# askerlee/AdaFace-dev

Measured on AMD Instinct MI355X. Metric: denoise-steps/sec SD-1.5 U-Net 512px bs=4/GPU, higher is better.
Workload: dtype f16; 1 GPU; adaface_txt2img_ddim: SD-1.5 U-Net eps-prediction + CFG + DDIM update, 512x512 (latent 64x64), bs=4/GPU, U-Net batch 8 (cond+uncond), 77 tokens, DDIM-50 timesteps, random-init weights; parallelism=replicas x1, hipgraph=True, finite=True

## Files before the change

### adaface-dev_amd/csrc/af_gemm.hip

```cpp
#include "af_common.h"

int af_gemm_n_major(int M, int N, int K, int cin) { return (long)N * K > (long)M * cin ? 1 : 0; }

namespace {

struct GemmDev {
  const half_t* a1;
  const half_t* a2;
  const half_t* wt;
  const float* bias;
  const half_t* rowbias;
  const half_t* residual;
  half_t* out;
  half_t* out2;
  int M, N, K, kpad;
  int c1, c2, lda1, lda2;
  int H, W, Ho, Wo, HoWo, Heff, Weff, stride, upsample;
  int rows_per_batch, ld_rowbias, act_silu, ld_out, split_col, ld_out2;
  int tiles_n, tiles_m, n_major;
  int tap_shift;
  int splits, kt_per_split;
  float* ws;
  int* counters;
  int out_f32;
  int wpf, wpf_coop;
};

constexpr int BK = 64;
enum { EPI_STD = 0, EPI_GEGLU = 1, EPI_SPLIT_T = 2 };

template <int BM, int BN, int TAPS, int EPI, bool FAST = false>
__global__ __launch_bounds__(256, 2) void af_gemm_kernel(GemmDev p) {
  constexpr int WM = BM / 2, WN = BN / 2;
  constexpr int TM = WM / 16, TN = WN / 16;
  constexpr int AI = BM / 32, WI = BN / 32;
  constexpr int STAGE = (BM + BN) * BK;
  extern __shared__ __attribute__((aligned(16))) char af_smem[];
  half_t* lds = reinterpret_cast<half_t*>(af_smem);

  const int tid = threadIdx.x, lane = tid & 63, wave = tid >> 6;
  const int wm = wave & 1, wn = wave >> 1;

  int tile_m, tile_n;
  {
    const int nwg = gridDim.x, bid = blockIdx.x;
    const int q = nwg >> 3, r = nwg & 7, xcd = bid & 7, idx = bid >> 3;
    const int lid = (xcd < r ? xcd * (q + 1) : r * (q + 1) + (xcd - r) * q) + idx;
    if (p.n_major) {
// ... 408 lines not shown
         ((uintptr_t)d->bias & 15) == 0 && (((uintptr_t)d->rowbias | (uintptr_t)d->residual) & 7) == 0 && d->ld_rowbias % 4 == 0 &&
         ((uintptr_t)d->out & (d->out_mode == AF_OUT_F32 ? 15 : 7)) == 0;
}

static int launch_direct(const GemmDev& p0, hipStream_t stream) {
  GemmDev p = p0;
  p.tiles_m = (p.M + 31) / 32;
  p.tiles_n = (p.N + 63) / 64;
  p.splits = 1;
  const dim3 grid(p.tiles_m * p.tiles_n), block(256);
  if ((p.kpad >> 5) % 4 == 0) hipLaunchKernelGGL(af_gemm_direct_kernel<4>, grid, block, 0, stream, p);
  else hipLaunchKernelGGL(af_gemm_direct_kernel<2>, grid, block, 0, stream, p);
  return af_check_launch("af_gemm(tile 18)");
}

__global__ __launch_bounds__(256) void af_splitk_reduce_kernel(GemmDev p) {
  const long i4 = (long)blockIdx.x * 256 + threadIdx.x;
  const int n4 = p.N >> 2;
  if (i4 >= (long)p.M * n4) return;
  const int m = (int)(i4 / n4);
  const int n0 = (int)(i4 - (long)m * n4) * 4;
  floatx4 v = {0.f, 0.f, 0.f, 0.f};
  for (int sp = 0; sp < p.splits; ++sp) v += *reinterpret_cast<const floatx4*>(p.ws + ((size_t)sp * p.M + m) * p.N + n0);
  if (p.bias) v += *reinterpret_cast<const floatx4*>(p.bias + n0);
  if (p.rowbias) {
    const half4_t rv = *reinterpret_cast<const half4_t*>(p.rowbias + (size_t)(m / p.rows_per_batch) * p.ld_rowbias + n0);
#pragma unroll
    for (int i = 0; i < 4; ++i) v[i] += (float)rv[i];
  }
  if (p.act_silu == 1) {
#pragma unroll
    for (int i = 0; i < 4; ++i) v[i] = af_silu(v[i]);
  } else if (p.act_silu == 3) {
#pragma unroll
    for (int i = 0; i < 4; ++i) v[i] = v[i] * af_sigmoid(1.702f * v[i]);
  }
  if (p.residual) {
    const half4_t rv = *reinterpret_cast<const half4_t*>(p.residual + (size_t)m * p.N + n0);
#pragma unroll
    for (int i = 0; i < 4; ++i) v[i] += (float)rv[i];
  }
  if (p.out_f32) {
    *reinterpret_cast<floatx4*>(reinterpret_cast<float*>(p.out) + (size_t)m * p.ld_out + n0) = v;
    return;
  }
  const half4_t h = {(half_t)v[0], (half_t)v[1], (half_t)v[2], (half_t)v[3]};
// ... 48 lines not shown
  if (cpg <= 0 || cpg % 2 != 0 || bn % cpg != 0 || N % cpg != 0 || N / cpg > 32 || N % bn != 0 || N % 8 != 0) return 0;
  if (rows_per_batch <= 0 || rows_per_batch % 128 != 0 || rows_per_batch / 128 > 128) return 0;
  return 1;
}

extern "C" int af_gemm(const af_gemm_desc* d, void* stream) {
  AF_REQUIRE(d != nullptr, "af_gemm: null descriptor");
  AF_REQUIRE(d->a1 && d->wt && d->out, "af_gemm: a1/wt/out must be non-null");
  AF_REQUIRE(d->M > 0 && d->N > 0 && d->K > 0, "af_gemm: M, N, K must be positive");
  AF_REQUIRE(d->taps == 1 || d->taps == 9, "af_gemm: taps must be 1 or 9");
  AF_REQUIRE(d->kpad % BK == 0 && d->kpad >= d->K, "af_gemm: kpad must be a multiple of 64 and >= K");
  AF_REQUIRE(d->N % 4 == 0, "af_gemm: N must be a multiple of 4");
  AF_REQUIRE(d->c1 > 0 && d->c1 % 8 == 0 && d->c2 >= 0 && d->c2 % 8 == 0, "af_gemm: c1/c2 must be multiples of 8");
  AF_REQUIRE(d->c2 == 0 || d->a2 != nullptr, "af_gemm: a2 is null but c2 > 0");
  const bool ktail = d->c3 > 0 || d->c4 > 0;
  if (ktail) {
    AF_REQUIRE(d->taps == 9 && d->c3 > 0 && d->a3 != nullptr && d->c4 >= 0 && (d->c4 == 0 || d->a4 != nullptr), "af_gemm: the K tail needs taps == 9 and a3 (a4 when c4 > 0)");
    AF_REQUIRE(d->c3 % 64 == 0 && d->c4 % 64 == 0, "af_gemm: c3 / c4 must be multiples of 64");
    AF_REQUIRE((d->lda3 == 0 || (d->lda3 >= d->c3 && d->lda3 % 8 == 0)) && (d->lda4 == 0 || (d->lda4 >= d->c4 && d->lda4 % 8 == 0)), "af_gemm: bad lda3 / lda4");
    AF_REQUIRE((d->stride == 0 || d->stride == 1) && d->upsample == 0 && d->tap_shift == 0, "af_gemm: the K tail needs stride 1, no upsample, no tap_shift");
    AF_SUPPORTED((d->tile >= 7 && d->tile <= 15), "af_gemm: the K tail runs on the whole-line tiles 7 .. 13, 15 and the halo-resident tile 14 only");
  }
  if (d->upsample == 3) {
    AF_SUPPORTED(d->tile == 14 && af_gemm_halo_variant(d) == 4, "af_gemm: upsample = 3 (phase form) runs on tile 14 inside af_gemm_halo_variant's scope only");
    AF_REQUIRE(d->zeros != nullptr, "af_gemm: zeros must be non-null");
    AfLaunchScope scope(AF_FAM_GEMM, stream);
    AF_SUPPORTED(af_gemm3_try_launch(d, 1, 11, (hipStream_t)stream) == 0, "af_gemm: upsample = 3 needs a 16-byte aligned output with ld_out % 8 == 0");
    return af_check_launch("af_gemm(tile 14, phase form)");
  }
  AF_REQUIRE(d->K == d->taps * (d->c1 + d->c2) + d->c3 + d->c4, "af_gemm: K != taps*(c1+c2) (+ c3 + c4)");
  const bool gnp = d->gn_partials != nullptr;
  if (gnp) {
    const int rpb = d->rows_per_batch > 0 ? d->rows_per_batch : d->M;
    AF_SUPPORTED(af_gemm_gn_stats_ok(d->tile, d->splits, d->taps, d->act, d->out_mode, d->N, d->gn_cpg, rpb) == 1,
                 "af_gemm: gn_partials needs a whole-line tile whose width is a multiple of gn_cpg, the standard fp16 epilogue, whole 128-row tiles per "
                 "batch item and no split-K (af_gemm_gn_stats_ok)");
    AF_REQUIRE(d->M % rpb == 0 && (d->ld_out == 0 || d->ld_out == d->N) && ((uintptr_t)d->out & 15) == 0, "af_gemm: gn_partials needs M = B * rows_per_batch and a dense, 16-byte aligned output");
  }
  GemmDev p;
  p.a1 = (const half_t*)d->a1;
  p.a2 = (const half_t*)d->a2;
  p.wt = (const half_t*)d->wt;
  p.bias = (const float*)d->bias;
  p.rowbias = (const half_t*)d->rowbias;
  p.residual = (const half_t*)d->residual;
  p.out = (half_t*)d->out;
  p.out2 = (half_t*)d->out2;
  p.M = d->M;
// ... 2 lines not shown
  p.kpad = d->kpad;
  p.c1 = d->c1;
  p.c2 = d->c2;
  p.lda1 = d->lda1 ? d->lda1 : d->c1;
  p.lda2 = d->lda2 ? d->lda2 : d->c2;
  p.stride = d->stride ? d->stride : 1;
  p.upsample = d->upsample;
  p.H = d->H;
  p.W = d->W;
  p.Ho = d->Ho;
  p.Wo = d->Wo;
  p.HoWo = d->Ho * d->Wo;
  p.Heff = p.upsample ? 2 * d->H : d->H;
  p.Weff = p.upsample ? 2 * d->W : d->W;
  if (p.upsample == 2 && d->taps == 9) {
    p.Heff = d->Ho;
    p.Weff = d->Wo;
  }
  p.rows_per_batch = d->rows_per_batch > 0 ? d->rows_per_batch : d->M;
  p.ld_rowbias = d->ld_rowbias;
  p.act_silu = d->act == AF_ACT_SILU ? 1 : (d->act == AF_ACT_QUICKGELU ? 3 : 0);
  p.split_col = d->split_col;
  p.ld_out2 = d->ld_out2;
  p.tiles_n = 0;
  p.tap_shift = d->taps == 9 ? d->tap_shift : 0;
  p.splits = d->splits > 1 ? d->splits : 1;
  p.kt_per_split = 0;
  p.ws = (float*)d->workspace;
  p.counters = (d->splitk_fused && d->workspace && d->workspace_bytes > AF_SPLITK_COUNTER_BYTES)
                   ? reinterpret_cast<int*>(static_cast<char*>(d->workspace) + d->workspace_bytes - AF_SPLITK_COUNTER_BYTES) : nullptr;
  if (d->taps == 9) {
    AF_REQUIRE(d->B > 0 && d->H > 0 && d->W > 0 && d->Ho > 0 && d->Wo > 0, "af_gemm: conv geometry missing");
    AF_REQUIRE(p.stride == 1 || p.stride == 2, "af_gemm: stride must be 1 or 2");
    AF_REQUIRE(p.upsample >= 0 && p.upsample <= 2, "af_gemm: upsample must be 0, 1 (nearest) or 2 (zero-insert)");
    AF_REQUIRE(!(p.upsample && p.stride != 1), "af_gemm: upsample requires stride 1");
    AF_REQUIRE(d->M == d->B * d->Ho * d->Wo, "af_gemm: M != B*Ho*Wo");
    if (p.upsample == 2)
      AF_REQUIRE((d->Ho == 2 * d->H || d->Ho == 2 * d->H - 1) && (d->Wo == 2 * d->W || d->Wo == 2 * d->W - 1),
                 "af_gemm: zero-insert mode needs Ho in {2H, 2H-1}, Wo in {2W, 2W-1}");
    AF_REQUIRE(d->Ho == (p.Heff + 2 - 3) / p.stride + 1 && d->Wo == (p.Weff + 2 - 3) / p.stride + 1,
               "af_gemm: Ho/Wo inconsistent with H/W/stride/upsample");
  }
  if (d->rowbias) AF_REQUIRE(d->ld_rowbias >= d->N, "af_gemm: ld_rowbias < N");
  const bool geglu = d->act == AF_ACT_GEGLU;
  if (geglu) {
    AF_REQUIRE(d->N % 32 == 0, "af_gemm: GEGLU needs N % 32 == 0 (interleaved 16-row groups)");
// ... 61 lines not shown
```

### adaface-dev_amd/csrc/af_gemm3.hip

```cpp
#include <algorithm>

#include "af_common.h"

int af_gemm_n_major(int M, int N, int K, int cin);

namespace {

struct Gemm3Dev {
  const half_t* a1;
  const half_t* a2;
  const half_t* wt;
  const half_t* zeros;
  const float* bias;
  const half_t* rowbias;
  const half_t* residual;
  half_t* out;
  half_t* out2;
  int split_col, ld_out2;
  int M, N, K, kpad, npad;
  int c1, c2, lda1, lda2;
  const half_t* a3;
  const half_t* a4;
  int c3, c4, lda3, lda4;
  int H, W, Ho, Wo, HoWo, stride;
// ... 724 lines not shown
    const int row = (wave * WPW + j) * 8 + prow;
    const int n = min(tile_n * BN + row, p.npad - 1);
    w_off[j] = ((unsigned)n * (unsigned)p.kpad + (unsigned)((slot ^ ((row >> 1) & 7)) * 8)) * 2u;
  }
  unsigned a_off1[APW], a_off2[APW];
  const half_t* a_px1[APW];
  const half_t* a_px2[APW];
#pragma unroll
  for (int j = 0; j < APW; ++j) {
    const int row = (wave * APW + j) * 8 + prow;
    const int mc = min(tile_m * BM + row, p.M - 1);
    const unsigned ch = (unsigned)(a_lc[j] * 8);
    if constexpr (TAPS == 9) {
      a_off1[j] = ((unsigned)mc * (unsigned)p.lda3 + ch) * 2u;
      a_off2[j] = ((unsigned)mc * (unsigned)p.lda4 + ch) * 2u;
      a_px1[j] = p.a1 + (size_t)a_base[j] * p.c1 + ch;
      a_px2[j] = p.a2 + (size_t)a_base[j] * p.c2 + ch;
    } else {
      a_off1[j] = ((unsigned)mc * (unsigned)p.lda1 + ch) * 2u;
      a_off2[j] = ((unsigned)mc * (unsigned)p.lda2 + ch) * 2u;
    }
  }

  auto issue_stage = [&](int kt, int sl) {
    char* As = af_smem + sl * STAGE;
    char* Ws = As + BM * 128;
    const int k0 = kt * BKW;
    if constexpr (TAPS == 9) {
      if (p.upsample) {
        const int tp = k0 / Cin;
        const int c0 = k0 - tp * Cin;
        const bool first = c0 < p.c1;
        const half_t* src = first ? p.a1 : p.a2;
        const int cs = first ? p.c1 : p.c2;
        const int coff = first ? c0 : c0 - p.c1;
        const int ty = tp / 3, tx = tp - ty * 3;
#pragma unroll
        for (int j = 0; j < APW; ++j) {
          const bool ok = (a_mask[j] >> tp) & 1u;
          const int dpix = (((a_par[j] & 1) + ty - 1) >> 1) * p.W + (((a_par[j] >> 1) + tx - 1) >> 1);
          const half_t* g = ok ? src + (size_t)(a_base[j] + dpix) * cs + coff + a_lc[j] * 8 : p.zeros;
          glds16(g, As + (wave * APW + j) * 1024);
        }
#pragma unroll
        for (int j = 0; j < WPW; ++j) glds16(wok[j] ? wptr[j] + k0 : p.zeros, Ws + (wave * WPW + j) * 1024);
        return;
      }
    }
    if (TAPS == 9 && p.c3 > 0 && k0 >= 9 * Cin) {
      const int kt0 = k0 - 9 * Cin;
      const bool first = kt0 < p.c3;
      const half_t* sb = first ? p.a3 + kt0 : p.a4 + (kt0 - p.c3);
      if (first) {
#pragma unroll
        for (int j = 0; j < APW; ++j) glds16_sbase(sb, a_off1[j], As + (wave * APW + j) * 1024);
      } else {
#pragma unroll
        for (int j = 0; j < APW; ++j) glds16_sbase(sb, a_off2[j], As + (wave * APW + j) * 1024);
      }
    } else if constexpr (TAPS == 9) {
      const int tp = k0 / Cin;
      const int c0 = k0 - tp * Cin;
      const bool first = c0 < p.c1;
      const int cs = first ? p.c1 : p.c2;
      const int ty = tp / 3, tx = tp - ty * 3;
      const long soff = (long)((ty - 1) * p.W + (tx - 1)) * cs + (first ? c0 : c0 - p.c1);
#pragma unroll
      for (int j = 0; j < APW; ++j) {
        const bool ok = (a_mask[j] >> tp) & 1u;
        const half_t* px = a_px1[j];
        if (!first) px = a_px2[j];
        const half_t* g = ok ? px + soff : p.zeros;
        glds16(g, As + (wave * APW + j) * 1024);
      }
    } else {
      const bool first = k0 < p.c1;
      const half_t* sb = first ? p.a1 + k0 : p.a2 + (k0 - p.c1);
      if (first) {
#pragma unroll
        for (int j = 0; j < APW; ++j) glds16_sbase(sb, a_off1[j], As + (wave * APW + j) * 1024);
      } else {
#pragma unroll
        for (int j = 0; j < APW; ++j) glds16_sbase(sb, a_off2[j], As + (wave * APW + j) * 1024);
      }
    }
// ... 741 lines not shown
      mfmas();
      __builtin_amdgcn_s_setprio(1);
      tb = tn_;
    }
    asm volatile("s_waitcnt vmcnt(0)" ::: "memory");
    __builtin_amdgcn_s_barrier();
  }
  __builtin_amdgcn_s_setprio(0);
  gemm3_epilogue<E3_STD, NWM, NWN, TN, CH_LDS, UP2 ? 2 : (PATCH ? 1 : 0)>(p, acc, af_smem, tile_m, tile_n, wm, wn, fr, fq, tid);
}

static bool conv3h_up2_ok(const af_gemm_desc* d) {
  if (d->taps != 9 || d->tap_shift || (d->stride ? d->stride : 1) != 1 || d->c1 <= 0 || d->c1 % 64 != 0 || d->c2 || d->c3 || d->c4) return false;
  if (d->N <= 0 || d->N % CH_BN != 0 || d->K != 4 * d->c1 || d->kpad % 64 != 0 || d->kpad < d->K) return false;
  if ((d->W != 16 && d->W != 32) || d->H <= 0 || d->B <= 0 || (d->H * d->W) % CH_BM != 0 || d->Ho != 2 * d->H || d->Wo != 2 * d->W) return false;
  if ((long)d->M != (long)d->B * d->Ho * d->Wo || d->splits > 1) return false;
  if (d->act == AF_ACT_GEGLU || d->out_mode != AF_OUT_NORMAL || d->ln_colsum != nullptr) return false;
  if (d->rowbias != nullptr || d->residual != nullptr || d->gn_partials != nullptr) return false;
  if ((long)d->B * d->H * d->W * d->c1 * 2 >= (1L << 32)) return false;
  if ((long)((4L * d->N + 127) / 128 * 128) * d->kpad * 2 >= (1L << 32)) return false;
  return true;
}

static int conv3h_variant(const af_gemm_desc* d) {
  if (d->upsample == 3) return conv3h_up2_ok(d) ? 4 : 0;
  if (d->taps != 9 || (d->upsample != 0 && d->upsample != 1) || d->tap_shift || d->c1 % 64 != 0 || d->c2 % 64 != 0) return 0;
  const bool n160 = d->N % CH_BN == 0;
  if (!n160 && d->N % 128 != 0) return 0;
  if (d->c3 || d->c4) {
    if (!n160 || d->c3 <= 0 || d->c3 % 64 != 0 || d->c4 < 0 || d->c4 % 64 != 0 || d->upsample) return 0;
    if ((long)d->M * std::max(d->lda3 ? d->lda3 : d->c3, d->lda4 ? d->lda4 : d->c4) * 2 >= (1L << 32)) return 0;
    if ((long)d->B * d->H * d->W >= (1L << 24)) return 0;
  }
  const int up = d->upsample ? 2 : 1;
  if ((d->stride ? d->stride : 1) != 1 || d->Ho != up * d->H || d->Wo != up * d->W) return 0;
  if (d->M % CH_BM != 0 || d->M != d->B * d->Ho * d->Wo) return 0;
  if (d->act == AF_ACT_GEGLU || d->out_mode == AF_OUT_SPLIT_T || d->ln_colsum != nullptr || d->kpad % 64 != 0) return 0;
  if ((long)d->B * d->H * d->W * std::max(d->c1, d->c2) * 2 >= (1L << 32)) return 0;
  if ((long)((d->N + 127) / 128 * 128) * d->kpad * 2 >= (1L << 32)) return 0;
  if (d->Wo > 64) {
    if (n160 || d->Wo % 16 != 0 || d->Ho % 16 != 0 || d->c3 || d->c4 || d->splits > 1) return 0;
    return 3;
  }
  if (d->Wo != 8 && d->Wo != 16 && d->Wo != 32 && d->Wo != 64) return 0;
  const int rows = CH_BM / d->Wo;
  if (d->Ho % rows != 0 && rows % d->Ho != 0) return 0;
  if (d->Ho < rows && (rows / d->Ho) * (d->Ho + 2) * (d->Wo + 2) > CH_NP_MAX * 8) return 0;
  return n160 ? 1 : 2;
// ... 288 lines not shown
          for (int tm = 0; tm < TM; ++tm) xf[tm] = *reinterpret_cast<const half8_t*>(As + (wm * 64 + tm * 16) * 128 + rd);
#pragma unroll
          for (int tn = 0; tn < 5; ++tn)
#pragma unroll
            for (int tm = 0; tm < TM; ++tm) acc3[tn][tm] = __builtin_amdgcn_mfma_f32_16x16x32_f16(wf[tn], xf[tm], acc3[tn][tm], 0, 0, 0);
        }
      }
    }
    gemm3_epilogue<E3_STD, 2, 4, 5, FF_XS + 2 * FF_W1S + FF_W2B>(p.epi_p, acc3, af_smem, tile_m, 0, wm, wn, fr, fq, tid, nullptr);
  }
}

}

extern "C" int af_gemm_halo_variant(const af_gemm_desc* d) { return d != nullptr ? conv3h_variant(d) : 0; }

int af_gemm3_try_launch(const af_gemm_desc* d, int splits, int wide, hipStream_t stream) {
  const bool geglu = d->act == AF_ACT_GEGLU, split_t = d->out_mode == AF_OUT_SPLIT_T;
  const bool halo_r5 = wide == 16;
  if (halo_r5) wide = 11;
  const int halo_variant = wide == 11 ? conv3h_variant(d) : 0;
  if (wide == 11 && halo_variant == 0) return 1;
  if (halo_r5 && (d->c3 > 0 || halo_variant != 1)) return 1;
  if (d->upsample == 3 && halo_variant != 4) return 1;
  if (d->upsample && d->upsample != 3 && !((wide == 4 || wide == 5 || (wide >= 8 && wide <= 12)) && d->upsample == 1 && d->taps == 9)) return 1;
  if (d->c1 % BK3 != 0 || d->c2 % BK3 != 0 || d->zeros == nullptr) return 1;
  if (d->c3 > 0 && (wide < 4 || (wide > 10 && wide != 12 && wide != 11) || d->taps != 9 || d->upsample || (d->stride != 0 && d->stride != 1))) return 1;
  if ((geglu || split_t) && (d->taps != 1 || splits > 1)) return 1;
  if (geglu && (!wide || d->N % (wide == 5 ? 128 : 256) != 0)) return 1;
  if (!geglu && wide == 1 && d->N % 320 != 0) return 1;
  if (wide >= 4) {
    if (d->c1 % 64 != 0 || d->c2 % 64 != 0 || d->kpad % 64 != 0) return 1;
    if (wide == 4 && (geglu ? d->N % 256 != 0 : d->N % 320 != 0)) return 1;
    if (wide == 5 && geglu && d->N % 128 != 0) return 1;
    if (wide == 6 && (!geglu || d->N % 320 != 0)) return 1;
    if (wide == 7 && (!geglu || d->N % 256 != 0)) return 1;
    if ((wide == 8 || wide == 10) && (geglu || split_t || d->N % 160 != 0)) return 1;
    if (wide == 9 && (geglu || split_t)) return 1;
    if (wide == 12 && (geglu || split_t || d->N % 128 != 0)) return 1;
    if (wide == 13 && (geglu || d->N % 128 != 0 || d->c3 > 0)) return 1;
    if (wide == 14 && (geglu || d->N % 64 != 0 || d->c3 > 0)) return 1;
    if (wide > 14) return 1;
  }
  if (wide == 2 && (d->N % 256 != 0 || d->taps != 1 || split_t || splits > 1)) return 1;
  if (wide == 3 && (d->N % 320 != 0 || d->taps != 1 || split_t || splits > 1)) return 1;
  if (d->ln_colsum != nullptr && (wide < 4 || d->taps != 1 || d->c2 != 0 || splits > 1)) return 1;
  if (d->gn_partials != nullptr && !((wide == 4 || wide == 8 || wide == 10 || wide == 11) && !geglu && !split_t && splits <= 1)) return 1;
// ... 34 lines not shown
  p.W = d->W;
  p.Ho = d->Ho;
  p.Wo = d->Wo;
  p.HoWo = d->Ho * d->Wo;
  p.stride = d->stride ? d->stride : 1;
  p.upsample = d->upsample;
  p.rows_per_batch = d->rows_per_batch > 0 ? d->rows_per_batch : d->M;
  p.ld_rowbias = d->ld_rowbias;
  p.act = d->act == AF_ACT_SILU ? 1 : (d->act == AF_ACT_QUICKGELU ? 3 : 0);
  p.ld_out = d->ld_out ? d->ld_out : (geglu ? d->N / 2 : (split_t ? d->split_col : d->N));
  p.tiles_n = 0;
  const int nk = p.kpad / BK3;
  p.splits = splits > 1 ? splits : 1;
  if (p.splits > nk) p.splits = nk;
  p.kt_per_split = (nk + p.splits - 1) / p.splits;
  p.splits = (nk + p.kt_per_split - 1) / p.kt_per_split;
  p.ws = (float*)d->workspace;
  p.counters = (d->splitk_fused && d->workspace && d->workspace_bytes > AF_SPLITK_COUNTER_BYTES)
                   ? reinterpret_cast<int*>(static_cast<char*>(d->workspace) + d->workspace_bytes - AF_SPLITK_COUNTER_BYTES) : nullptr;
  p.wpf = 0;
  p.wpf_coop = 1;
  static const int ablate = getenv("AF_GEMM3_ABLATE") ? atoi(getenv("AF_GEMM3_ABLATE")) : 0;
  p.ablate = ablate & (128 | 256);
  {
    const long ldmax = std::max(std::max((long)(d->lda1 ? d->lda1 : d->c1), (long)(d->lda2 ? d->lda2 : d->c2)), std::max((long)(d->lda3 ? d->lda3 : d->c3), (long)(d->lda4 ? d->lda4 : d->c4)));
    if (wide >= 4 && wide != 11 && (long)d->M * ldmax * 2 >= (1L << 32)) return 1;
    if (wide >= 4 && wide != 11 && (long)p.npad * p.kpad * 2 >= (1L << 32)) return 1;
  }
  {
    const int ncols = geglu ? d->N / 2 : d->N;
    p.stage_ok = ncols % 8 == 0 && p.ld_out % 8 == 0 && (reinterpret_cast<uintptr_t>(p.out) & 15) == 0;
  }
  if (wide == 11) {
    const int nchunk = conv3h_chunks(d);
    p.splits = splits > 1 ? splits : 1;
    if (p.splits > nchunk) p.splits = nchunk;
    p.kt_per_split = (nchunk + p.splits - 1) / p.splits;
    p.splits = (nchunk + p.kt_per_split - 1) / p.kt_per_split;
    if (halo_variant == 3) {
      if (!p.stage_ok) return 1;
      p.splits = 1;
    }
    if (halo_variant == 4) {
      if (!p.stage_ok || splits > 1) return 1;
      p.up2_cout = d->N;
      p.N = 4 * d->N;
// ... 160 lines not shown
```

### adaface-dev_amd/ldm/modules/attention.py

```python
import math
import os as _os

import torch
import torch.nn as nn
import torch.nn.functional as F

from ... import ops
from ...ops import AF_ACT_GEGLU, F16
from .diffusionmodules.util import (Conv2d, GroupNorm32, LayerNorm, Linear, _PackCache, checkpoint, from_nhwc_f16,
                                    to_nhwc_f16, zero_module)


FOLD_LAYERNORM = _os.environ.get("AF_FOLD_LAYERNORM", "1") != "0"
FUSE_GN_PROJ = _os.environ.get("AF_FUSE_GN_PROJ", "1") != "0"
CHAIN_XATTN = _os.environ.get("AF_CHAIN_XATTN", "1") != "0"
XATTN_FUSE_MIN_TOKENS = int(_os.environ.get("AF_XATTN_FUSE_MIN_TOKENS", "8192"))
CHAIN_PROJ_OUT = _os.environ.get("AF_CHAIN_PROJ_OUT", "1") != "0"
FUSE_XATTN640 = _os.environ.get("AF_FUSE_XATTN640", "0") != "0"
XATTN640_FUSE_MIN_TOKENS = 4096
FUSE_XATTN = _os.environ.get("AF_FUSE_XATTN", "1") != "0"
FUSE_FF = _os.environ.get("AF_FUSE_FF", "1") != "0"


def exists(val):
    return val is not None


def default(val, d):
    if exists(val):
        return val
    return d() if callable(d) else d


def Normalize(in_channels):
    return GroupNorm32(num_groups=32, num_channels=in_channels, eps=1e-6, affine=True)


class GEGLU(nn.Module):

    def __init__(self, dim_in, dim_out):
        super().__init__()
# ... 41 lines not shown

    def forward(self, x):
        y = self.hip(x.reshape(-1, x.shape[-1]).to(F16).contiguous())
        y = y.reshape(*x.shape[:-1], y.shape[-1])
        return y if x.dtype == F16 else y.to(x.dtype)


class FeedForward(nn.Module):
    def __init__(self, dim, dim_out=None, mult=4, glu=False, dropout=0.0):
        super().__init__()
        inner_dim = int(dim * mult)
        dim_out = default(dim_out, dim)
        if not glu:
            raise NotImplementedError("FeedForward(glu=False) is not on the SD-1.5 path")
        if dropout != 0.0:
            raise NotImplementedError("dropout > 0 is not supported (SD-1.5 uses 0)")
        self.net = nn.Sequential(GEGLU(dim, inner_dim), nn.Dropout(dropout), Linear(inner_dim, dim_out))

    def ff_fusable(self, M, C, ln) -> bool:
        return bool(FUSE_FF and ln is not None and C == 320 and M >= 24576)

    def hip(self, x2d, residual=None, ln=None, post=None):
        if post is not None:
            pw_p, x_in, rpb, cpg = post
            return ops.ff_chain(x2d, self.net[0].packed_ln(ln), self.net[2].packed(), residual, pw_p, x_in, rows_per_batch=rpb, gn_cpg=cpg)
        if FUSE_FF and ln is not None and x2d.shape[1] == 320 and x2d.shape[0] >= 24576:
            return ops.ff_fused(x2d, self.net[0].packed_ln(ln), self.net[2].packed(), residual=residual)
        return self.net[2].hip(self.net[0].hip(x2d, ln=ln), residual=residual)

    def hip_train(self, x2d, residual=None, ln=None):
        g, hp = self.net[0].hip_train(x2d, ln=ln)
        return self.net[2].hip(g, residual=residual), hp

    def hip_bwd(self, hp, dy):
        return self.net[0].hip_bwd(hp, self.net[2].hip_dgrad(dy))

    def forward(self, x):
        y = self.hip(x.reshape(-1, x.shape[-1]).to(F16).contiguous()).reshape(x.shape[:-1] + (-1,))
        return y if x.dtype == F16 else y.to(x.dtype)


class CrossAttention(nn.Module):

    def __init__(self, query_dim, context_dim=None, heads=8, dim_head=64, dropout=0.0):
        super().__init__()
        inner_dim = dim_head * heads
        context_dim = default(context_dim, query_dim)
        if dropout != 0.0:
# ... 149 lines not shown
        self.ff = FeedForward(dim, dropout=dropout, glu=gated_ff)
        self.attn2 = CrossAttention(query_dim=dim, context_dim=context_dim, heads=n_heads, dim_head=d_head, dropout=dropout)
        self.norm1 = LayerNorm(dim)
        self.norm2 = LayerNorm(dim)
        self.norm3 = LayerNorm(dim)
        self.checkpoint = checkpoint

    def hip(self, x2d, B, N, context=None, keybias=None, post=None):
        if FOLD_LAYERNORM and x2d.shape[1] % 64 == 0:
            small = x2d.shape[0] < 1024
            if (CHAIN_XATTN and not small and context is not None and not self.attn1.save_cross_attn_vars 
                    and self.attn2.xattn_fusable(x2d.shape[1], B, N, context.shape[1], self.norm2, chain=True)):
                pre = self.attn1.hip(x2d, B, N, None, keybias, residual=x2d, ln=self.norm1, defer_out=True)
                x2 = self.attn2.hip(None, B, N, context, None, residual=None, ln=self.norm2, pre=pre)
                return self.ff.hip(x2, residual=x2, ln=self.norm3, post=post if self.post_done(x2d.shape[0], x2d.shape[1], post) else None)
            x1 = self.attn1.hip(self.norm1.hip(x2d) if small else x2d, B, N, None, keybias, residual=x2d, ln=None if small else self.norm1)
            x2 = self.attn2.hip(self.norm2.hip(x1) if small else x1, B, N, context, None, residual=x1, ln=None if small else self.norm2)
            return self.ff.hip(x2, residual=x2, ln=self.norm3, post=post if self.post_done(x2d.shape[0], x2d.shape[1], post) else None)
        x1 = self.attn1.hip(self.norm1.hip(x2d), B, N, None, keybias, residual=x2d)
        x2 = self.attn2.hip(self.norm2.hip(x1), B, N, context, None, residual=x1)
        return self.ff.hip(self.norm3.hip(x2), residual=x2)

    def post_done(self, M, C, post) -> bool:
        return bool(post is not None and CHAIN_PROJ_OUT and FOLD_LAYERNORM and C % 64 == 0 and self.ff.ff_fusable(M, C, self.norm3))

    def hip_train(self, x2d, B, N, context=None, keybias=None):
        if FOLD_LAYERNORM and x2d.shape[1] % 64 == 0 and x2d.shape[0] >= 1024:
            x1, s1 = self.attn1.hip_train(x2d, B, N, None, keybias, residual=x2d, ln=self.norm1)
            x2, s2 = self.attn2.hip_train(x1, B, N, context, None, residual=x1, ln=self.norm2)
            x3, hp = self.ff.hip_train(x2, residual=x2, ln=self.norm3)
            return x3, (x2d, x1, x2, s1, s2, hp)
        x1, s1 = self.attn1.hip_train(self.norm1.hip(x2d), B, N, None, keybias, residual=x2d)
        x2, s2 = self.attn2.hip_train(self.norm2.hip(x1), B, N, context, None, residual=x1)
        x3, hp = self.ff.hip_train(self.norm3.hip(x2), residual=x2)
        return x3, (x2d, x1, x2, s1, s2, hp)

    def hip_bwd(self, saved, dy, dctx=None):
        x, x1, x2, s1, s2, hp = saved
        dx2 = self.norm3.hip_bwd(x2, self.ff.hip_bwd(hp, dy), add=dy)
        dn2, dctx = self.attn2.hip_bwd(s2, dx2, dctx)
        dx1 = self.norm2.hip_bwd(x1, dn2, add=dx2)
        dn1, _ = self.attn1.hip_bwd(s1, dx1, None)
        return self.norm1.hip_bwd(x, dn1, add=dx1), dctx

    def forward(self, x, context=None, mask=None):
        return checkpoint(self._forward, (x, context, mask), self.parameters(), self.checkpoint)

# ... 7 lines not shown

class SpatialTransformer(nn.Module):

    def __init__(self, in_channels, n_heads, d_head, depth=1, dropout=0.0, context_dim=None):
        super().__init__()
        self.in_channels = in_channels
        inner_dim = n_heads * d_head
        self.norm = Normalize(in_channels)
        self.proj_in = Conv2d(in_channels, inner_dim, kernel_size=1, stride=1, padding=0)
        self.transformer_blocks = nn.ModuleList(
            [BasicTransformerBlock(inner_dim, n_heads, d_head, dropout=dropout, context_dim=context_dim) for _ in range(depth)]
        )
        self.proj_out = zero_module(Conv2d(inner_dim, in_channels, kernel_size=1, stride=1, padding=0))

    live_mask_rule = False

    def _keybias(self, mask, B, H, W):
        m2 = F.interpolate(mask.float(), size=(H, W), mode="nearest")
        kb = ops.make_keybias(m2.reshape(B, H * W), H * W)
        if self.live_mask_rule:
            any_empty = (m2.sum(dim=(2, 3)) == 0).any()
            kb = torch.where(any_empty, torch.zeros_like(kb), kb)
        return kb

    def hip(self, x, context=None, mask=None):
        B, H, W, Cn = x.shape
        N = H * W
        y = ops.gn_proj_fused(x, self.norm.weight, self.norm.bias, self.norm.eps, self.proj_in.packed(), self.norm.num_groups) if FUSE_GN_PROJ else None
        if y is None:
            y = self.norm.hip(x)
            y = self.proj_in.hip(y).reshape(B * N, -1)
        kb = None
        if mask is not None:
            kb = self._keybias(mask, B, H, W)
        cpg = Cn // 32 if Cn % 32 == 0 else 0
        last = len(self.transformer_blocks) - 1
        post = (self.proj_out.packed(), x.reshape(B * N, Cn), N, cpg)
        chained = False
        for i, block in enumerate(self.transformer_blocks):
            block.attn2.infeat_size = (H, W)
            if i == last and block.post_done(B * N, y.shape[1], post):
                y, chained = block.hip(y, B, N, context, kb, post=post), True
            else:
                y = block.hip(y, B, N, context, kb)
        out = y if chained else ops.gemm(y, self.proj_out.packed(), residual=x.reshape(B * N, Cn), rows_per_batch=N, gn_cpg=cpg)
        out4 = out.reshape(B, H, W, Cn)
        if hasattr(out, "_gn_partials"):
            out4._gn_partials = out._gn_partials
        return out4

    def hip_train(self, x, context=None, mask=None):
        B, H, W, Cn = x.shape
        N = H * W
        y, st = self.norm.hip_train(x)
        y = self.proj_in.hip(y).reshape(B * N, -1)
        kb = None
        if mask is not None:
            kb = self._keybias(mask, B, H, W)
        bs = []
        for block in self.transformer_blocks:
# ... 19 lines not shown
```

### adaface-dev_amd/ldm/modules/diffusionmodules/util.py

```python

import os

import numpy as np
import torch
import torch.nn as nn

from .... import ops
from ....ops import F16


def to_nhwc_f16(x: torch.Tensor, cpad: int = 0) -> torch.Tensor:
    if x.dtype == F16 and cpad <= x.shape[1] and x.is_contiguous(memory_format=torch.channels_last):
        return x.permute(0, 2, 3, 1)
    return ops.nchw_f32_to_nhwc_f16(x, cpad)


def from_nhwc_f16(y: torch.Tensor, dtype: torch.dtype, channels: int = 0) -> torch.Tensor:
    channels = channels or y.shape[-1]
    if dtype == F16 and channels == y.shape[-1]:
        return y.permute(0, 3, 1, 2)
    out = ops.nhwc_f16_to_nchw_f32(y, channels)
    return out if dtype == torch.float32 else out.to(dtype)


# ... 40 lines not shown
            raise NotImplementedError(f"Conv2d kernel={ks} stride={st} padding={pd}: only 3x3/pad1/stride1|2 and 1x1 are on the hot path")
        self._cache = _PackCache()
        self.cin_pad = 0

    def packed(self) -> ops.PackedWeight:
        _require_cuda(self.weight, "Conv2d")

        def build():
            if self.kernel_size == (3, 3):
                return ops.pack_conv3x3(self.weight, self.bias, self.weight.device, self.cin_pad)
            return ops.pack_matrix(self.weight.detach().reshape(self.out_channels, self.in_channels), self.bias, self.weight.device)

        return self._cache.get((self.weight, self.bias), build)

    def packed_up2(self) -> ops.PackedWeight:
        _require_cuda(self.weight, "Conv2d")
        if not hasattr(self, "_cache_up2"):
            self._cache_up2 = _PackCache()
        return self._cache_up2.get((self.weight, self.bias), lambda: ops.pack_conv3x3_up2(self.weight, self.bias, self.weight.device))

    def hip(self, x, x2=None, upsample=False, rowbias=None, residual=None, gn_groups=0):
        if upsample is True and self.kernel_size == (3, 3) and self.stride[0] == 1 and not gn_groups and os.environ.get("AF_UP2_PHASE", "1") != "0":
            B, H, W, c1 = x.shape
            d = ops.conv_up2_desc(B, H, W, c1, self.out_channels, c2=0 if x2 is None else x2.shape[-1], rowbias=rowbias, residual=residual)
            if ops.conv_up2_eligible(d):
                return ops.conv3x3_up2(x, self.packed_up2(), tile=14, splits=1)
        pw = self.packed()
        cpg = self.out_channels // gn_groups if gn_groups and self.out_channels % gn_groups == 0 else 0
        if self.kernel_size == (3, 3):
            return ops.conv3x3(x, pw, x2=x2, stride=self.stride[0], upsample=upsample, rowbias=rowbias, residual=residual, gn_cpg=cpg)
        B, H, W, c1 = x.shape
        a2 = None if x2 is None else x2.reshape(B * H * W, x2.shape[-1])
        res = None if residual is None else residual.reshape(B * H * W, -1)
        out = ops.gemm(x.reshape(B * H * W, c1), pw, a2=a2, rowbias=rowbias, rows_per_batch=H * W, residual=res, gn_cpg=cpg)
        out4 = out.reshape(B, H, W, -1)
        if hasattr(out, "_gn_partials"):
            out4._gn_partials = out._gn_partials
        return out4

    def packed_bwd(self) -> ops.PackedWeight:
        _require_cuda(self.weight, "Conv2d")

        def build():
            w = self.weight.detach()
            if self.kernel_size == (3, 3):
                wd = w.flip(2, 3).permute(1, 0, 2, 3).contiguous()
                return ops.pack_conv3x3(wd, None, w.device, ops.round_up(self.out_channels, 8))
            return ops.pack_matrix(w.reshape(self.out_channels, self.in_channels).t().contiguous(), None, w.device)

# ... 158 lines not shown
```

### adaface-dev_amd/ops.py

```python
import ctypes as C
from dataclasses import dataclass
from typing import Optional

import torch

from . import _lib
from ._lib import AF_ACT_GEGLU, AF_ACT_NONE, AF_ACT_QUICKGELU, AF_ACT_SILU, AF_OUT_F32, AF_OUT_NORMAL, AF_OUT_SPLIT_T, GemmDesc

F16 = torch.float16
NEG_MAX = -torch.finfo(torch.float32).max



def param_key(p):
    if p is None:
        return None
    gen = p.__dict__.get("_af_gen")
    return (p.data_ptr(), p._version, p.device, gen[0] if gen is not None else -1)


def _stream() -> int:
    return torch._C._cuda_getCurrentRawStream(torch._C._cuda_getDevice())


# ... 86 lines not shown
            b = b + b3.detach().float()
        if b1 is not None:
            b = b + b1.detach().float().to(b.device)
    pw = pack_matrix(w, b, device, taps=9, cin=cin)
    pw.k_tail = cs
    return pw


def up2_phase_weights(w: torch.Tensor) -> torch.Tensor:
    cout, cin, kh, kw = w.shape
    assert kh == 3 and kw == 3
    fold = w.new_zeros((2, 2, 3))
    fold[0, 0, 0] = fold[0, 1, 1] = fold[0, 1, 2] = 1
    fold[1, 0, 0] = fold[1, 0, 1] = fold[1, 1, 2] = 1
    return torch.einsum("pai,qbj,ocij->pqoabc", fold, fold, w).reshape(4, cout, 2, 2, cin)


def pack_conv3x3_up2(w: torch.Tensor, bias: Optional[torch.Tensor], device) -> PackedWeight:
    cout, cin = w.shape[:2]
    wp = up2_phase_weights(w.detach().to(device=device, dtype=torch.float32)).reshape(4 * cout, 4 * cin)
    pw = pack_matrix(wp, bias, device, taps=9, cin=cin)
    pw.N, pw.up2 = cout, True
    return pw


def interleave_geglu(w: torch.Tensor, b: torch.Tensor):
    inner = w.shape[0] // 2
    assert inner % 16 == 0
    wv, wg = w[:inner].reshape(inner // 16, 16, -1), w[inner:].reshape(inner // 16, 16, -1)
    wi = torch.stack([wv, wg], dim=1).reshape(2 * inner, -1)
    bv, bg = b[:inner].reshape(inner // 16, 16), b[inner:].reshape(inner // 16, 16)
    bi = torch.stack([bv, bg], dim=1).reshape(2 * inner)
    return wi, bi


import json as _json
import os as _os

_TUNE_PATH = _os.environ.get("AF_TUNE_TABLE") or _os.path.join(_os.path.dirname(_os.path.abspath(__file__)), "tuning", "gfx950_gemm.json")
_tune_table = None
def conv_halo_eligible(d) -> bool:
    return _lib.lib().af_gemm_halo_variant(C.byref(d)) != 0


_tune_recorder = None
_splitk_ws = {}
# ... 282 lines not shown
        assert residual.shape == out.shape
    if skip is not None:
        s1, s2 = skip
        assert stride == 1 and not upsample and not tap_shift and (ho, wo) == (H, W)
        _chk_f16(s1, "conv3x3.skip")
        assert s1.shape[:3] == out.shape[:3]
        c3, c4 = s1.shape[3], 0
        if s2 is not None:
            _chk_f16(s2, "conv3x3.skip2")
            assert s2.shape[:3] == out.shape[:3]
            c4 = s2.shape[3]
        assert c3 + c4 == pw.k_tail, f"conv3x3: skip channels {c3}+{c4} vs the packed tail {pw.k_tail}"
        d.a3, d.a4, d.c3, d.c4, d.lda3, d.lda4 = _p(s1), _p(s2), c3, c4, c3, c4
        if tile == 0 and splits == 0 and _tune_recorder is None:
            tile, splits = conv3x3_skip_tile(d.M, d.N, c1 + c2, pw.k_tail)
            if tile == 14 and not conv_halo_eligible(d):
                tile, splits = _whole_line_tile(d.M, d.N), 1
    gn = _launch_gemm(d, x.device, "af_gemm(conv3x3)", tile, splits, gn_cpg=gn_cpg)
    if gn is not None:
        gn.attach(out)
    return out


def conv_up2_desc(B: int, H: int, W: int, c1: int, cout: int, *, c2: int = 0, rowbias=None, residual=None, splits: int = 1) -> "GemmDesc":
    d = GemmDesc()
    d.rowbias, d.residual = _p(rowbias), _p(residual)
    d.M, d.N, d.K, d.kpad, d.taps = B * 4 * H * W, cout, 4 * c1, round_up(4 * c1, 64), 9
    d.c1, d.c2 = c1, c2
    d.B, d.H, d.W, d.Ho, d.Wo = B, H, W, 2 * H, 2 * W
    d.stride, d.upsample = 1, 3
    d.rows_per_batch = 4 * H * W
    d.ld_rowbias = 0 if rowbias is None else rowbias.stride(0)
    d.splits = splits
    return d


def conv_up2_eligible(d) -> bool:
    return _lib.lib().af_gemm_halo_variant(C.byref(d)) == 4


def conv3x3_up2(x: torch.Tensor, pw: PackedWeight, *, tile: int = 14, splits: int = 1) -> torch.Tensor:
    _chk_f16(x, "conv3x3_up2.x")
    B, H, W, c1 = x.shape
    assert pw.up2 and pw.cin == c1, f"conv3x3_up2: needs a pack_conv3x3_up2 weight of {c1} input channels"
    out = torch.empty((B, 2 * H, 2 * W, pw.N), dtype=F16, device=x.device)
    d = conv_up2_desc(B, H, W, c1, pw.N)
    assert d.K == pw.K and d.kpad == pw.kpad
    d.a1, d.wt, d.bias, d.out = _p(x), _p(pw.wt), _p(pw.bias), _p(out)
    _launch_gemm(d, x.device, "af_gemm(conv3x3_up2)", tile, splits)
    return out


def ff_fused(x2d: torch.Tensor, pw1: PackedWeight, pw2: PackedWeight, residual: Optional[torch.Tensor] = None) -> torch.Tensor:
    _chk_f16(x2d, "ff_fused.x")
    M, Cn = x2d.shape
    assert pw1.K == Cn and pw2.N == Cn and pw2.K * 2 == pw1.N and pw1.bias is not None
    out = torch.empty((M, Cn), dtype=F16, device=x2d.device)
    if residual is not None:
        _chk_f16(residual, "ff_fused.residual")
        assert residual.shape == out.shape
    _pf_note(pw1.wt, pw2.wt)
    _launch("af_ff_fused", _p(x2d), _p(pw1.wt), _p(pw1.bias), _p(pw1.ln_cs), float(pw1.ln_eps), pw1.kpad, _p(pw2.wt), _p(pw2.bias), pw2.kpad,
            _p(residual), _p(out), M, Cn, pw2.K, _p(_zero_page(x2d.device)))
    return out


def ff_chain(x2d: torch.Tensor, pw1: PackedWeight, pw2: PackedWeight, residual: torch.Tensor, pw_p: PackedWeight, x_in: torch.Tensor, *, rows_per_batch: int,
             gn_cpg: int = 0) -> torch.Tensor:
    _chk_f16(x2d, "ff_chain.x")
# ... 1050 lines not shown
```

Baseline: 101.9 denoise-steps/s.

## Fold feed-forward output linear into proj_out and add split-K phase-form upsample conv

For transformer blocks whose feed-forward cannot use the fused chain, the second feed-forward linear and proj_out are algebraically folded into one GEMM. Its packed weight is [Wp·W2 | Wp] with a combined bias, and it consumes the GEGLU output plus the residual as a second A operand. This removes one GEMM launch and the intermediate activation round-trip, at the cost of a larger K and an fp16 product weight that may shift numerics slightly. A split-K path for the 2x phase-form upsample conv at 8x8 is also added, using a whole-line tile and a reduce kernel that scatters the phases. That path stays behind an environment flag that is off by default.

```diff
diff --git a/adaface-dev_amd/csrc/af_gemm.hip b/adaface-dev_amd/csrc/af_gemm.hip
--- a/adaface-dev_amd/csrc/af_gemm.hip
+++ b/adaface-dev_amd/csrc/af_gemm.hip
@@ -24,6 +24,7 @@
   int* counters;
   int out_f32;
   int wpf, wpf_coop;
+  int up2_cout;
 };
 
 constexpr int BK = 64;
@@ -478,6 +479,15 @@
   const int n0 = (int)(i4 - (long)m * n4) * 4;
   floatx4 v = {0.f, 0.f, 0.f, 0.f};
   for (int sp = 0; sp < p.splits; ++sp) v += *reinterpret_cast<const floatx4*>(p.ws + ((size_t)sp * p.M + m) * p.N + n0);
+  if (p.up2_cout > 0) {
+    const int ph = n0 / p.up2_cout, ch = n0 - ph * p.up2_cout;
+    const int hw = p.H * p.W, b = m / hw, rem = m - b * hw, y = rem / p.W, x = rem - y * p.W;
+    const size_t row = ((size_t)b * 2 * p.H + 2 * y + (ph >> 1)) * 2 * p.W + 2 * x + (ph & 1);
+    if (p.bias) v += *reinterpret_cast<const floatx4*>(p.bias + ch);
+    const half4_t h = {(half_t)v[0], (half_t)v[1], (half_t)v[2], (half_t)v[3]};
+    *reinterpret_cast<half4_t*>(p.out + row * p.ld_out + ch) = h;
+    return;
+  }
   if (p.bias) v += *reinterpret_cast<const floatx4*>(p.bias + n0);
   if (p.rowbias) {
     const half4_t rv = *reinterpret_cast<const half4_t*>(p.rowbias + (size_t)(m / p.rows_per_batch) * p.ld_rowbias + n0);
@@ -572,8 +582,34 @@
     AF_SUPPORTED((d->tile >= 7 && d->tile <= 15), "af_gemm: the K tail runs on the whole-line tiles 7 .. 13, 15 and the halo-resident tile 14 only");
   }
   if (d->upsample == 3) {
-    AF_SUPPORTED(d->tile == 14 && af_gemm_halo_variant(d) == 4, "af_gemm: upsample = 3 (phase form) runs on tile 14 inside af_gemm_halo_variant's scope only");
+    const int hv = af_gemm_halo_variant(d);
+    AF_SUPPORTED((d->tile == 14 && hv == 4) || hv == 5, "af_gemm: upsample = 3 (phase form) runs inside af_gemm_halo_variant's scope only: tile 14, or a whole-line "
+                                                        "tile under split-K at the 8 x 8 level");
     AF_REQUIRE(d->zeros != nullptr, "af_gemm: zeros must be non-null");
+    if (hv == 5) {
+      const int eff = af_gemm3_effective_splits(d, d->splits, d->tile - 3);
+      AF_REQUIRE(eff >= 2 && d->workspace != nullptr && d->workspace_bytes >= (int64_t)eff * d->M * d->N * 4,
+                 "af_gemm: the phase form on a whole-line tile needs split-K and workspace >= splits*M*N*4 bytes");
+      const int ldo = d->ld_out ? d->ld_out : d->N;
+      AF_REQUIRE(ldo >= d->N && ldo % 4 == 0 && ((uintptr_t)d->out & 7) == 0 && ((uintptr_t)d->bias & 15) == 0, "af_gemm: upsample = 3 needs an 8-byte aligned output with ld_out % 4 == 0");
+      AfLaunchScope scope(AF_FAM_GEMM, stream);
+      AF_SUPPORTED(af_gemm3_try_launch(d, d->splits, d->tile - 3, (hipStream_t)stream) == 2, "af_gemm: upsample = 3 is outside the chosen whole-line tile's scope");
+      GemmDev r{};
+      r.ws = (float*)d->workspace;
+      r.bias = (const float*)d->bias;
+      r.out = (half_t*)d->out;
+      r.M = d->B * d->H * d->W;
+      r.N = 4 * d->N;
+      r.H = d->H;
+      r.W = d->W;
+      r.up2_cout = d->N;
+      r.ld_out = ldo;
+      r.splits = eff;
+      r.rows_per_batch = r.M;
+      const long n = (long)r.M * (r.N >> 2);
+      hipLaunchKernelGGL(af_splitk_reduce_kernel, dim3((unsigned)((n + 255) / 256)), dim3(256), 0, (hipStream_t)stream, r);
+      return af_check_launch("af_gemm(phase form, split-K)");
+    }
     AfLaunchScope scope(AF_FAM_GEMM, stream);
     AF_SUPPORTED(af_gemm3_try_launch(d, 1, 11, (hipStream_t)stream) == 0, "af_gemm: upsample = 3 needs a 16-byte aligned output with ld_out % 8 == 0");
     return af_check_launch("af_gemm(tile 14, phase form)");
@@ -622,6 +658,7 @@
   p.act_silu = d->act == AF_ACT_SILU ? 1 : (d->act == AF_ACT_QUICKGELU ? 3 : 0);
   p.split_col = d->split_col;
   p.ld_out2 = d->ld_out2;
+  p.up2_cout = 0;
   p.tiles_n = 0;
   p.tap_shift = d->taps == 9 ? d->tap_shift : 0;
   p.splits = d->splits > 1 ? d->splits : 1;
diff --git a/adaface-dev_amd/csrc/af_gemm3.hip b/adaface-dev_amd/csrc/af_gemm3.hip
--- a/adaface-dev_amd/csrc/af_gemm3.hip
+++ b/adaface-dev_amd/csrc/af_gemm3.hip
@@ -770,6 +770,14 @@
     }
   }
 
+  int up2_tap0 = 0;
+  if constexpr (TAPS == 9) {
+    if (p.up2_cout > 0) {
+      const int ph = (tile_n * BN) / p.up2_cout;
+      up2_tap0 = (ph >> 1) * 3 + (ph & 1);
+    }
+  }
+
   auto issue_stage = [&](int kt, int sl) {
     char* As = af_smem + sl * STAGE;
     char* Ws = As + BM * 128;
@@ -807,8 +815,9 @@
         for (int j = 0; j < APW; ++j) glds16_sbase(sb, a_off2[j], As + (wave * APW + j) * 1024);
       }
     } else if constexpr (TAPS == 9) {
-      const int tp = k0 / Cin;
-      const int c0 = k0 - tp * Cin;
+      const int kq = k0 / Cin;
+      const int c0 = k0 - kq * Cin;
+      const int tp = p.up2_cout > 0 ? up2_tap0 + (kq >> 1) * 3 + (kq & 1) : kq;
       const bool first = c0 < p.c1;
       const int cs = first ? p.c1 : p.c2;
       const int ty = tp / 3, tx = tp - ty * 3;
@@ -1596,8 +1605,21 @@
   return true;
 }
 
+static bool conv3w_up2_ok(const af_gemm_desc* d) {
+  if (d->taps != 9 || d->tap_shift || (d->stride ? d->stride : 1) != 1 || d->c1 <= 0 || d->c1 % 64 != 0 || d->c2 || d->c3 || d->c4) return false;
+  const int bn = d->tile == 7 ? 320 : ((d->tile == 11 || d->tile == 13) ? 160 : ((d->tile == 8 || d->tile == 12) ? 128 : 0));
+  if (bn == 0 || d->N <= 0 || d->N % bn != 0 || d->K != 4 * d->c1 || d->kpad != d->K) return false;
+  if (d->W != 8 || d->H != 8 || d->B <= 0 || d->Ho != 2 * d->H || d->Wo != 2 * d->W || (long)d->M != (long)d->B * d->Ho * d->Wo) return false;
+  if (d->splits < 2 || d->splits > 16 || d->splits > d->kpad / 64) return false;
+  if (d->act != AF_ACT_NONE || d->out_mode != AF_OUT_NORMAL || d->ln_colsum != nullptr) return false;
+  if (d->rowbias != nullptr || d->residual != nullptr || d->gn_partials != nullptr) return false;
+  if ((long)d->M * d->c1 * 2 >= (1L << 32)) return false;
+  if ((long)((4L * d->N + 127) / 128 * 128) * d->kpad * 2 >= (1L << 32)) return false;
+  return true;
+}
+
 static int conv3h_variant(const af_gemm_desc* d) {
-  if (d->upsample == 3) return conv3h_up2_ok(d) ? 4 : 0;
+  if (d->upsample == 3) return conv3h_up2_ok(d) ? 4 : (conv3w_up2_ok(d) ? 5 : 0);
   if (d->taps != 9 || (d->upsample != 0 && d->upsample != 1) || d->tap_shift || d->c1 % 64 != 0 || d->c2 % 64 != 0) return 0;
   const bool n160 = d->N % CH_BN == 0;
   if (!n160 && d->N % 128 != 0) return 0;
@@ -1932,7 +1954,8 @@
   const int halo_variant = wide == 11 ? conv3h_variant(d) : 0;
   if (wide == 11 && halo_variant == 0) return 1;
   if (halo_r5 && (d->c3 > 0 || halo_variant != 1)) return 1;
-  if (d->upsample == 3 && halo_variant != 4) return 1;
+  const bool up2w = d->upsample == 3 && wide != 11 && d->tile == wide + 3 && splits == d->splits && conv3h_variant(d) == 5;
+  if (d->upsample == 3 && halo_variant != 4 && !up2w) return 1;
   if (d->upsample && d->upsample != 3 && !((wide == 4 || wide == 5 || (wide >= 8 && wide <= 12)) && d->upsample == 1 && d->taps == 9)) return 1;
   if (d->c1 % BK3 != 0 || d->c2 % BK3 != 0 || d->zeros == nullptr) return 1;
   if (d->c3 > 0 && (wide < 4 || (wide > 10 && wide != 12 && wide != 11) || d->taps != 9 || d->upsample || (d->stride != 0 && d->stride != 1))) return 1;
@@ -2013,6 +2036,17 @@
   p.wpf_coop = 1;
   static const int ablate = getenv("AF_GEMM3_ABLATE") ? atoi(getenv("AF_GEMM3_ABLATE")) : 0;
   p.ablate = ablate & (128 | 256);
+  if (up2w) {
+    p.up2_cout = d->N;
+    p.M = d->B * d->H * d->W;
+    p.N = 4 * d->N;
+    p.npad = (p.N + 127) / 128 * 128;
+    p.Ho = d->H;
+    p.Wo = d->W;
+    p.HoWo = d->H * d->W;
+    p.upsample = 0;
+    p.counters = nullptr;
+  }
   {
     const long ldmax = std::max(std::max((long)(d->lda1 ? d->lda1 : d->c1), (long)(d->lda2 ? d->lda2 : d->c2)), std::max((long)(d->lda3 ? d->lda3 : d->c3), (long)(d->lda4 ? d->lda4 : d->c4)));
     if (wide >= 4 && wide != 11 && (long)d->M * ldmax * 2 >= (1L << 32)) return 1;
diff --git a/adaface-dev_amd/ldm/modules/attention.py b/adaface-dev_amd/ldm/modules/attention.py
--- a/adaface-dev_amd/ldm/modules/attention.py
+++ b/adaface-dev_amd/ldm/modules/attention.py
@@ -16,7 +16,8 @@
 CHAIN_XATTN = _os.environ.get("AF_CHAIN_XATTN", "1") != "0"
 XATTN_FUSE_MIN_TOKENS = int(_os.environ.get("AF_XATTN_FUSE_MIN_TOKENS", "8192"))
 CHAIN_PROJ_OUT = _os.environ.get("AF_CHAIN_PROJ_OUT", "1") != "0"
-FUSE_XATTN640 = _os.environ.get("AF_FUSE_XATTN640", "0") != "0"
+FOLD_PROJ_OUT = _os.environ.get("AF_FOLD_PROJ_OUT", "1") != "0"
+FUSE_XATTN640 =_os.environ.get("AF_FUSE_XATTN640", "0") != "0"
 XATTN640_FUSE_MIN_TOKENS = 4096
 FUSE_XATTN = _os.environ.get("AF_FUSE_XATTN", "1") != "0"
 FUSE_FF = _os.environ.get("AF_FUSE_FF", "1") != "0"
@@ -104,8 +105,10 @@
 
     def hip(self, x2d, residual=None, ln=None, post=None):
         if post is not None:
-            pw_p, x_in, rpb, cpg = post
-            return ops.ff_chain(x2d, self.net[0].packed_ln(ln), self.net[2].packed(), residual, pw_p, x_in, rows_per_batch=rpb, gn_cpg=cpg)
+            pw_p, x_in, rpb, cpg, fold = post
+            if self.ff_fusable(x2d.shape[0], x2d.shape[1], ln):
+                return ops.ff_chain(x2d, self.net[0].packed_ln(ln), self.net[2].packed(), residual, pw_p, x_in, rows_per_batch=rpb, gn_cpg=cpg)
+            return ops.gemm(self.net[0].hip(x2d, ln=ln), fold(), a2=residual, residual=x_in, rows_per_batch=rpb, gn_cpg=cpg)
         if FUSE_FF and ln is not None and x2d.shape[1] == 320 and x2d.shape[0] >= 24576:
             return ops.ff_fused(x2d, self.net[0].packed_ln(ln), self.net[2].packed(), residual=residual)
         return self.net[2].hip(self.net[0].hip(x2d, ln=ln), residual=residual)
@@ -301,7 +304,11 @@
         return self.ff.hip(self.norm3.hip(x2), residual=x2)
 
     def post_done(self, M, C, post) -> bool:
-        return bool(post is not None and CHAIN_PROJ_OUT and FOLD_LAYERNORM and C % 64 == 0 and self.ff.ff_fusable(M, C, self.norm3))
+        if post is None or not FOLD_LAYERNORM or C % 64 != 0:
+            return False
+        if self.ff.ff_fusable(M, C, self.norm3):
+            return CHAIN_PROJ_OUT
+        return bool(FOLD_PROJ_OUT and post[4] is not None)
 
     def hip_train(self, x2d, B, N, context=None, keybias=None):
         if FOLD_LAYERNORM and x2d.shape[1] % 64 == 0 and x2d.shape[0] >= 1024:
@@ -355,6 +362,13 @@
             any_empty = (m2.sum(dim=(2, 3)) == 0).any()
             kb = torch.where(any_empty, torch.zeros_like(kb), kb)
         return kb
+
+    def _packed_ff_proj_out(self):
+        lin = self.transformer_blocks[-1].ff.net[2]
+        if not hasattr(self, "_fold_cache"):
+            self._fold_cache = _PackCache()
+        return self._fold_cache.get((lin.weight, lin.bias, self.proj_out.weight, self.proj_out.bias),
+                                    lambda: ops.pack_ff_proj_out(lin.weight, lin.bias, self.proj_out.weight, self.proj_out.bias, lin.weight.device))
 
     def hip(self, x, context=None, mask=None):
         B, H, W, Cn = x.shape
@@ -368,7 +382,7 @@
             kb = self._keybias(mask, B, H, W)
         cpg = Cn // 32 if Cn % 32 == 0 else 0
         last = len(self.transformer_blocks) - 1
-        post = (self.proj_out.packed(), x.reshape(B * N, Cn), N, cpg)
+        post = (self.proj_out.packed(), x.reshape(B * N, Cn), N, cpg, self._packed_ff_proj_out)
         chained = False
         for i, block in enumerate(self.transformer_blocks):
             block.attn2.infeat_size = (H, W)
diff --git a/adaface-dev_amd/ldm/modules/diffusionmodules/util.py b/adaface-dev_amd/ldm/modules/diffusionmodules/util.py
--- a/adaface-dev_amd/ldm/modules/diffusionmodules/util.py
+++ b/adaface-dev_amd/ldm/modules/diffusionmodules/util.py
@@ -86,9 +86,11 @@
     def hip(self, x, x2=None, upsample=False, rowbias=None, residual=None, gn_groups=0):
         if upsample is True and self.kernel_size == (3, 3) and self.stride[0] == 1 and not gn_groups and os.environ.get("AF_UP2_PHASE", "1") != "0":
             B, H, W, c1 = x.shape
-            d = ops.conv_up2_desc(B, H, W, c1, self.out_channels, c2=0 if x2 is None else x2.shape[-1], rowbias=rowbias, residual=residual)
-            if ops.conv_up2_eligible(d):
-                return ops.conv3x3_up2(x, self.packed_up2(), tile=14, splits=1)
+            tile, splits = ops.conv_up2_config(B, H, W, c1, self.out_channels)
+            d = ops.conv_up2_desc(B, H, W, c1, self.out_channels, c2=0 if x2 is None else x2.shape[-1], rowbias=rowbias, residual=residual,
+                                  tile=tile, splits=splits)
+            if ops.conv_up2_eligible(d) and (tile == 14 or os.environ.get("AF_UP2_PHASE_8X8", "0") != "0"):
+                return ops.conv3x3_up2(x, self.packed_up2(), tile=tile, splits=splits)
         pw = self.packed()
         cpg = self.out_channels // gn_groups if gn_groups and self.out_channels % gn_groups == 0 else 0
         if self.kernel_size == (3, 3):
diff --git a/adaface-dev_amd/ops.py b/adaface-dev_amd/ops.py
--- a/adaface-dev_amd/ops.py
+++ b/adaface-dev_amd/ops.py
@@ -132,6 +132,21 @@
     pw = pack_matrix(wp, bias, device, taps=9, cin=cin)
     pw.N, pw.up2 = cout, True
     return pw
+
+
+def pack_ff_proj_out(w2: torch.Tensor, b2: Optional[torch.Tensor], wp: torch.Tensor, bp: Optional[torch.Tensor], device) -> PackedWeight:
+    w2f = w2.detach().to(device=device, dtype=torch.float32)
+    wpf = wp.detach().to(device=device, dtype=torch.float32).reshape(wp.shape[0], -1)
+    assert wpf.shape[1] == w2f.shape[0], f"pack_ff_proj_out: proj_out takes {wpf.shape[1]} channels, the feed-forward gives {w2f.shape[0]}"
+    b = None
+    if b2 is not None:
+        b = (wpf * b2.detach().to(device=device, dtype=torch.float32)[None, :]).sum(dim=1)
+    if bp is not None:
+        bpf = bp.detach().to(device=device, dtype=torch.float32)
+        b = bpf if b is None else b + bpf
+    rows = max(1, (1 << 26) // (wpf.shape[1] * w2f.shape[1]))
+    prod = torch.cat([(wpf[i:i + rows, :, None] * w2f[None, :, :]).sum(dim=1) for i in range(0, wpf.shape[0], rows)], dim=0)
+    return pack_matrix(torch.cat([prod, wpf], dim=1), b, device)
 
 
 def interleave_geglu(w: torch.Tensor, b: torch.Tensor):
@@ -460,8 +475,16 @@
     return out
 
 
-def conv_up2_desc(B: int, H: int, W: int, c1: int, cout: int, *, c2: int = 0, rowbias=None, residual=None, splits: int = 1) -> "GemmDesc":
+UP2_SPLITK_SHAPES = {(2048, 1280, 5120): (7, 4)}
+
+
+def conv_up2_config(B: int, H: int, W: int, c1: int, cout: int):
+    return UP2_SPLITK_SHAPES.get((B * 4 * H * W, cout, 4 * c1), (14, 1)) if (H, W) == (8, 8) else (14, 1)
+
+
+def conv_up2_desc(B: int, H: int, W: int, c1: int, cout: int, *, c2: int = 0, rowbias=None, residual=None, tile: int = 14, splits: int = 1) -> "GemmDesc":
     d = GemmDesc()
+    d.tile = tile
     d.rowbias, d.residual = _p(rowbias), _p(residual)
     d.M, d.N, d.K, d.kpad, d.taps = B * 4 * H * W, cout, 4 * c1, round_up(4 * c1, 64), 9
     d.c1, d.c2 = c1, c2
@@ -474,15 +497,19 @@
 
 
 def conv_up2_eligible(d) -> bool:
-    return _lib.lib().af_gemm_halo_variant(C.byref(d)) == 4
-
-
-def conv3x3_up2(x: torch.Tensor, pw: PackedWeight, *, tile: int = 14, splits: int = 1) -> torch.Tensor:
+    return _lib.lib().af_gemm_halo_variant(C.byref(d)) in (4, 5)
+
+
+def conv3x3_up2(x: torch.Tensor, pw: PackedWeight, *, tile: int = 14, splits: int = 1, out: Optional[torch.Tensor] = None) -> torch.Tensor:
     _chk_f16(x, "conv3x3_up2.x")
     B, H, W, c1 = x.shape
     assert pw.up2 and pw.cin == c1, f"conv3x3_up2: needs a pack_conv3x3_up2 weight of {c1} input channels"
-    out = torch.empty((B, 2 * H, 2 * W, pw.N), dtype=F16, device=x.device)
-    d = conv_up2_desc(B, H, W, c1, pw.N)
+    if out is None:
+        out = torch.empty((B, 2 * H, 2 * W, pw.N), dtype=F16, device=x.device)
+    else:
+        _chk_f16(out, "conv3x3_up2.out")
+        assert tuple(out.shape) == (B, 2 * H, 2 * W, pw.N), f"conv3x3_up2: out must be {(B, 2 * H, 2 * W, pw.N)}, got {tuple(out.shape)}"
+    d = conv_up2_desc(B, H, W, c1, pw.N, tile=tile, splits=splits)
     assert d.K == pw.K and d.kpad == pw.kpad
     d.a1, d.wt, d.bias, d.out = _p(x), _p(pw.wt), _p(pw.bias), _p(out)
     _launch_gemm(d, x.device, "af_gemm(conv3x3_up2)", tile, splits)
```

Result: faster. 103.0 denoise-steps/s, median of 6 (+1.2%).
